# mx-strk/InformationBottleneckDecodingLDPC

Measured on AMD Instinct MI355X. Metric: decoded codewords/sec + achieved HBM GB/s, DVB-S2 N=64800 i_max=50, higher is better.
Workload: dtype u4

## Files before the change

### include/ibldpc.h

```cpp
#ifndef IBLDPC_H
#define IBLDPC_H

#include <stdint.h>

#ifdef __cplusplus
extern "C" {
#endif

#define IBL_VERSION 3

enum { IBL_OK = 0, IBL_EINVAL = -1, IBL_EHIP = -2, IBL_ENOMEM = -3, IBL_EUNSUPPORTED = -4 };
enum { IBL_U8 = 1, IBL_I32 = 2, IBL_F32 = 3, IBL_F64 = 4, IBL_I8 = 5 };
enum { IBL_MINSUM = 0, IBL_BP = 1 };
enum { IBL_PATH_AUTO = 0, IBL_PATH_PASSES = 1, IBL_PATH_FUSED = 2 };
enum { IBL_FLAG_FORCE_GENERIC = 1 };

typedef struct ibl_graph ibl_graph;
typedef struct ibl_ib ibl_ib;
typedef struct ibl_float ibl_float;

int ibl_version(void);
const char* ibl_last_error(void);
int ibl_device_count(int32_t* n);

// ... 6 lines not shown
int ibl_graph_info(const ibl_graph* g, int32_t* n_v, int32_t* n_c, int64_t* n_e, int32_t* d_c_max,
                   int32_t* d_v_max);
void ibl_graph_destroy(ibl_graph* g);

int ibl_ib_create(const ibl_graph* g, int32_t T_ch, int32_t T_dec, int32_t imax,
                  const int32_t* cn_lut, int64_t cn_len, const int32_t* vn_lut, int64_t vn_len,
                  const int32_t* match_cn, int64_t mc_len, const int32_t* match_vn, int64_t mv_len,
                  int32_t match, int32_t max_batch, int32_t flags, ibl_ib** out);
int ibl_ib_path(const ibl_ib* h);
int ibl_ib_set_path(ibl_ib* h, int32_t path);
int ibl_ib_path_in_use(const ibl_ib* h, int32_t* fused);
int ibl_ib_set_small_batch(ibl_ib* h, int32_t max_b);
int ibl_ib_small_batch(const ibl_ib* h, int32_t* max_b);
int ibl_ib_folded(const ibl_ib* h, int32_t* n_folded);
int ibl_ib_set_fold(ibl_ib* h, int32_t on);
int ibl_ib_fused_ncw(const ibl_ib* h, int32_t B, int32_t* ncw);
int ibl_ib_decode(ibl_ib* h, const void* d_ch, int32_t ch_dtype, int32_t B, void* d_out, int32_t out_dtype,
                  int32_t early_stop, int32_t* d_iters, void* stream);
void ibl_ib_destroy(ibl_ib* h);
int ibl_ib_timing(ibl_ib* h, int32_t enable);
int ibl_ib_timing_read(ibl_ib* h, double* cn_ms, int32_t* cn_launches, double* vn_ms, int32_t* vn_launches);

int ibl_float_create(const ibl_graph* g, int32_t kind, int32_t imax, double llr_max, int32_t precision,
                     int32_t max_batch, ibl_float** out);
int ibl_float_decode(ibl_float* h, const void* d_llr, int32_t llr_dtype, int32_t B, void* d_out,
                     int32_t out_dtype, int32_t early_stop, int32_t* d_iters, void* stream);
void ibl_float_destroy(ibl_float* h);
int ibl_float_set_path(ibl_float* h, int32_t path);
int ibl_float_path_in_use(const ibl_float* h, int32_t* fused);
int ibl_float_fused_geometry(const ibl_float* h, int32_t B, int32_t* ngroups, int32_t* grid);
// ... 66 lines not shown
```

### informationbottleneckdecodingldpc_amd/_lib.py

```python
from __future__ import annotations

import ctypes
import os

import numpy as np

_HERE = os.path.dirname(os.path.abspath(__file__))
LIB_PATH = os.environ.get("IBLDPC_LIB") or os.path.join(_HERE, "libibldpc.so")

IBL_OK, IBL_EINVAL, IBL_EHIP, IBL_ENOMEM, IBL_EUNSUPPORTED = 0, -1, -2, -3, -4
IBL_U8, IBL_I32, IBL_F32, IBL_F64, IBL_I8 = 1, 2, 3, 4, 5
IBL_MINSUM, IBL_BP = 0, 1
IBL_FLAG_FORCE_GENERIC = 1
IBL_PATH_AUTO, IBL_PATH_PASSES, IBL_PATH_FUSED = 0, 1, 2

EXPORTS = [
    "ibl_version", "ibl_last_error", "ibl_device_count", "ibl_map_node_connections",
    "ibl_graph_create", "ibl_graph_info", "ibl_graph_destroy",
    "ibl_ib_create", "ibl_ib_path", "ibl_ib_set_path", "ibl_ib_path_in_use", "ibl_ib_fused_ncw", "ibl_ib_decode",
    "ibl_ib_set_small_batch", "ibl_ib_small_batch", "ibl_ib_folded", "ibl_ib_set_fold",
    "ibl_ib_destroy",
    "ibl_float_create", "ibl_float_decode", "ibl_float_destroy", "ibl_count_below",
    "ibl_float_set_path", "ibl_float_path_in_use", "ibl_float_fused_geometry", "ibl_float_folded",
    "ibl_float_input_check",
    "ibl_float_set_small_batch", "ibl_float_small_batch",
    "ibl_float_create_corrected", "ibl_float_correction",
    "ibl_ib_timing", "ibl_ib_timing_read", "ibl_float_timing", "ibl_float_timing_read",
    "ibl_channel_sample",
    "ibl_encoder_create",
    "ibl_encoder_algorithm",
    "ibl_encode",
    "ibl_encoder_destroy",
    "ibl_random_bits",
    "ibl_count_errors",
    "ibl_shard_range", "ibl_comm_unique_id", "ibl_comm_create", "ibl_comm_broadcast", "ibl_comm_allreduce_sum_i64",
# ... 30 lines not shown
    L.ibl_graph_create.argtypes = [_i32, _i32, _i32p, _i32p, _i32, ctypes.POINTER(_vp)]
    L.ibl_graph_info.argtypes = [_vp, ctypes.POINTER(_i32), ctypes.POINTER(_i32), ctypes.POINTER(_i64),
                                 ctypes.POINTER(_i32), ctypes.POINTER(_i32)]
    L.ibl_graph_destroy.argtypes = [_vp]
    L.ibl_graph_destroy.restype = None
    L.ibl_ib_create.argtypes = [_vp, _i32, _i32, _i32, _i32p, _i64, _i32p, _i64, _i32p, _i64, _i32p, _i64,
                                _i32, _i32, _i32, ctypes.POINTER(_vp)]
    L.ibl_ib_path.argtypes = [_vp]
    L.ibl_ib_set_path.argtypes = [_vp, _i32]
    L.ibl_ib_path_in_use.argtypes = [_vp, ctypes.POINTER(_i32)]
    L.ibl_ib_fused_ncw.argtypes = [_vp, _i32, ctypes.POINTER(_i32)]
    L.ibl_ib_set_small_batch.argtypes = [_vp, _i32]
    L.ibl_ib_small_batch.argtypes = [_vp, ctypes.POINTER(_i32)]
    L.ibl_ib_folded.argtypes = [_vp, ctypes.POINTER(_i32)]
    L.ibl_ib_set_fold.argtypes = [_vp, _i32]
    L.ibl_ib_decode.argtypes = [_vp, _vp, _i32, _i32, _vp, _i32, _i32, _vp, _vp]
    L.ibl_ib_destroy.argtypes = [_vp]
    L.ibl_ib_destroy.restype = None
    L.ibl_float_create.argtypes = [_vp, _i32, _i32, ctypes.c_double, _i32, _i32, ctypes.POINTER(_vp)]
    L.ibl_float_decode.argtypes = [_vp, _vp, _i32, _i32, _vp, _i32, _i32, _vp, _vp]
    L.ibl_float_destroy.argtypes = [_vp]
    L.ibl_float_destroy.restype = None
    L.ibl_float_set_path.argtypes = [_vp, _i32]
    L.ibl_float_path_in_use.argtypes = [_vp, ctypes.POINTER(_i32)]
    L.ibl_float_fused_geometry.argtypes = [_vp, _i32, ctypes.POINTER(_i32), ctypes.POINTER(_i32)]
    L.ibl_float_folded.argtypes = [_vp, ctypes.POINTER(_i32)]
    L.ibl_float_set_small_batch.argtypes = [_vp, _i32]
    L.ibl_float_small_batch.argtypes = [_vp, ctypes.POINTER(_i32)]
    L.ibl_float_input_check.argtypes = [_vp, ctypes.POINTER(_i32), _vp]
    L.ibl_float_create_corrected.argtypes = [_vp, ctypes.c_double, ctypes.c_double, _i32, ctypes.c_double, _i32, _i32,
# ... 96 lines not shown
```

### informationbottleneckdecodingldpc_amd/csrc/capi_ib.hip

```cpp
#include <cstring>
#include <functional>

#include "host.h"

using namespace ibl;

struct ibl_ib {
  const ibl_graph* g = nullptr;
  int32_t Tc = 0, T = 0, imax = 0, CM = 0, VM = 0, match = 0, max_batch = 0, ldb = 0;
  bool fast = false;
  DevBuf<uint8_t> cin, vin, ch8;
  DevBuf<int32_t> flags, dL;
  DevBuf<uint32_t> cn_img, vn_img, dec_img;
  int cn_nt = 0, vn_nt = 0, dec_nt = 0;
  int32_t cn_fslot[kMaxD + 1] = {0}, vn_fslot[kMaxD + 1] = {0};
  KCfg kcn, kvn, kdec;
  KTimer timer;
  int32_t n_folded = 0, fold_slot = -1, n_rest = 0, rest_heavy = 0;
  bool fold_on = true;
  std::vector<int32_t> fold_rec, fold_cn_info, fold_vn_info;
  DevBuf<uint8_t> cin2;
  DevBuf<int32_t> fold, cn_info_f, vn_info_r;
  int32_t path = IBL_PATH_AUTO;
  bool fused_ok = false, f_half_ok = false;
  int32_t f_ncw_forced = 0;
  int32_t small_b = 0;
  bool s_ok = false;
  size_t s_lds_cn = 0, s_lds_vn = 0, s_lds_dec = 0;
  ChainGraphs s_graphs;
  FusedTaskBufs ft;
  int32_t f_nreg = 0, f_dbuf = 0, f_cn_uni = 0, f_vn_uni = 0;
  size_t f_lds = 0;
  int f_grid = 0, f_block = 0;
  DevBuf<int32_t> cn_lut, vn_lut, mc, mv;
  int64_t cn_len = 0, vn_len = 0, mc_len = 0, mv_len = 0;
};

// ... 226 lines not shown
  }
  if (const char* ne = getenv("IBL_FUSED_NCW")) h->f_ncw_forced = atoi(ne);
  h->f_nreg = nreg;
  h->f_dbuf = dbuf ? 1 : 0;
  h->f_lds = lds;
  h->f_block = block;
  h->f_grid = bpc * g->num_cus;
  h->fused_ok = true;
  return IBL_OK;
}

int ib_configure_fast(ibl_ib* h, const IbImages& im) {
  const ibl_graph* g = h->g;
  const int CM = h->CM, VM = h->VM;
  int rc;
  if ((rc = h->cn_img.upload(im.cn_img)) || (rc = h->vn_img.upload(im.vn_img)) || (rc = h->dec_img.upload(im.dec_img)))
    return rc;
  if ((rc = pick_cfg(0, CM, 4 * h->cn_nt, g->num_cus, &h->kcn)) ||
      (rc = pick_cfg(1, VM, 4 * h->vn_nt, g->num_cus, &h->kvn)) ||
      (rc = pick_cfg(2, VM, 4 * h->dec_nt, g->num_cus, &h->kdec)))
    return rc;
  size_t priv = 0;
  const char* kname = "";
  HIPCHK(ib_fast_private_bytes(CM, VM, &priv, &kname));
#if IBL_DIAG
  const bool allow_scratch = getenv("IBL_ALLOW_SCRATCH") != nullptr;
#else
  const bool allow_scratch = false;
#endif
  if (!allow_scratch && (rc = refuse_private(priv, std::string("fast-path kernel ") + kname + " has a ",
                                             "-byte private segment (register spill / scratch item): rebuild required")))
    return rc;
// ... 152 lines not shown
  dc.aligned = out_aligned(B, d_out, 4, out_dtype == kU8 ? 1 : 4);
  HIPCHK(launch_ib_dec_small(dc, grid_of(g->n_vn_task, h->s_lds_dec), h->s_lds_dec, s));
  return IBL_OK;
}

int ib_decode_fast(ibl_ib* h, const void* d_ch, int32_t ch_dtype, int32_t B, void* d_out, int32_t out_dtype,
                   bool early, int32_t* d_iters, hipStream_t s) {
  const ibl_graph* g = h->g;
  const int I = h->imax;
  const int ccn = ib_fast_chunk(h->CM), cvn = ib_fast_chunk(h->VM);
  const int ldbb = h->ldb / 2;
  HIPCHK(launch_ib_stage4(d_ch, ch_dtype, g->n_v, B, h->ch8, ldbb, s));
  IbFastArgs cn{}, vn{};
  ib_pass_args(h, B, ldbb, &cn, &vn);
  cn.n_heavy = g->cn_heavy; vn.n_heavy = g->vn_heavy;
  const bool fold = h->fold_on && h->n_folded > 0 && I > 1;
  int rc;
  if (fold) {
    if ((rc = ib_fold_alloc(h))) return rc;
    vn.info = h->vn_info_r; vn.n_nodes = h->n_rest; vn.n_heavy = h->rest_heavy;
    cn.fold = h->fold; cn.fold_slot = h->fold_slot;
  }
  uint8_t* cb[2] = {h->cin, fold ? h->cin2 : h->cin};
  auto cn_fold = [&](int j) {
    const bool f = fold && j < I - 1;
    cn.info = f ? h->cn_info_f.get() : g->cn_info.get();
    cn.fold_mode = f ? ((early && j >= 1) ? 2 : 1) : 0;
    cn.fout = f ? cb[(j + 1) & 1] : nullptr;
  };
#if IBL_DIAG
// ... 20 lines not shown
  const char* trace_path = getenv("IBL_TRACE_WAVES");
  TraceBuf tr;
  nwv = (size_t)h->kvn.grid * (h->kvn.block / 64);
  const size_t nwc = (size_t)h->kcn.grid * (h->kcn.block / 64);
  if (trace_path && I > 1) {
    if ((rc = tr.open(3 * (nwv + nwc), s))) return rc;
    trace = tr.d;
  }
#endif
  for (int j = 1; j < I; ++j) {
    const int32_t* gate = flag_row(h->flags, early && j >= 2, j - 1);
    vn.img = h->vn_img + (size_t)(j - 1) * h->vn_nt * 256;
    vn.gate = gate;
    vn.trace = (trace && j == I / 2) ? trace : nullptr;
    vn.out = cb[j & 1];
    HIPCHK(h->timer.timed(1, s, [&] { return launch_ib_vn_fast(vn, h->VM, h->kvn.grid, h->kvn.block, h->kvn.lds, s); }));
    cn.img = h->cn_img + (size_t)j * h->cn_nt * 256;
    cn.gate = gate;
    cn.unsat = flag_row(h->flags, early, j);
    cn.trace = (trace && j == I / 2) ? trace + 3 * nwv : nullptr;
    cn.in = cb[j & 1];
    cn_fold(j);
    HIPCHK(h->timer.timed(0, s, launch_cn));
  }
#if IBL_DIAG
  if (trace && ((rc = tr.save(s, std::string(trace_path) + "_vn.bin", 0, 3 * nwv)) ||
                (rc = tr.save(s, std::string(trace_path) + "_cn.bin", 3 * nwv, 3 * nwc))))
    return rc;
#endif
  HIPCHK(launch_finalize(h->flags, I, early ? 1 : 0, h->dL, d_iters, s));
  IbDecArgs dc{};
// ... 113 lines not shown
  return IBL_OK;
}

int ibl_ib_folded(const ibl_ib* h, int32_t* n_folded) {
  if (!h || !n_folded) return fail(IBL_EINVAL, "NULL argument");
  *n_folded = h->n_folded;
  return IBL_OK;
}

int ibl_ib_set_fold(ibl_ib* h, int32_t on) {
  if (!h) return fail(IBL_EINVAL, "decoder is NULL");
  h->fold_on = on != 0;
  return IBL_OK;
}

int ibl_ib_timing(ibl_ib* h, int32_t enable) { return timing_enable(h, enable); }
int ibl_ib_timing_read(ibl_ib* h, double* cn_ms, int32_t* cn_n, double* vn_ms, int32_t* vn_n) {
  return timing_read(h, cn_ms, cn_n, vn_ms, vn_n);
}

void ibl_ib_destroy(ibl_ib* h) {
  if (h) (void)hipSetDevice(h->g->device);
  delete h;
}

int ibl_ib_decode(ibl_ib* h, const void* d_ch, int32_t ch_dtype, int32_t B, void* d_out, int32_t out_dtype,
                  int32_t early_stop, int32_t* d_iters, void* stream) {
  if (!h) return fail(IBL_EINVAL, "decoder is NULL");
  if (B < 1 || B > h->max_batch) return fail(IBL_EINVAL, "B must lie in [1, max_batch]");
  if (ch_dtype != kU8 && ch_dtype != kI32) return fail(IBL_EINVAL, "channel dtype must be IBL_U8 or IBL_I32");
// ... 14 lines not shown
```

### informationbottleneckdecodingldpc_amd/csrc/common.h

```cpp
#pragma once
#include <hip/hip_runtime.h>
#pragma clang diagnostic ignored "-Wunused-result"
#include <stddef.h>
#include <stdint.h>

#include "plan.h"

namespace ibl {

constexpr int kWave = 64;
constexpr int kChunk = 256;
#ifndef IBL_W
#define IBL_W 2
#endif
constexpr int kW = IBL_W;
constexpr int kChunkIB = 512 * kW;
#ifndef IBL_LIGHT_W
#define IBL_LIGHT_W 4
#endif
constexpr int kRowPad = 512 * (IBL_LIGHT_W > IBL_W ? IBL_LIGHT_W : IBL_W);
constexpr int kChunkDec = 512;
constexpr int kTbl = 8192;
constexpr int kSuper = 65536;
constexpr int kRowSh = 12, kColSh = 8;
// ... 5 lines not shown
constexpr int kShards = 64;
constexpr int kLdsBytes = 160 * 1024;

enum Dtype : int32_t { kU8 = 1, kI32 = 2, kF32 = 3, kF64 = 4, kI8 = 5 };

int set_error(int code, const char* msg);

typedef __attribute__((address_space(4))) const int32_t cint32;
__device__ __forceinline__ int32_t sload(const int32_t* p, int i) { return ((cint32*)p)[i]; }

__device__ __forceinline__ int take_ticket(int* ctr, int lane) {
  int t = 0;
  if (lane == 0) t = __hip_atomic_fetch_add(ctr, 1, __ATOMIC_RELAXED, __HIP_MEMORY_SCOPE_WORKGROUP);
  return __builtin_amdgcn_readfirstlane(t);
}

struct IbFastArgs {
  const uint8_t* in;
  uint8_t* out;
  const uint8_t* ch8;
  const int32_t* info;
  const int32_t* tgt;
  const int32_t* gather;
  const uint32_t* img;
  const int32_t* gate;
  int32_t* unsat;
  int32_t fslot[kMaxD + 1];
  int32_t nt;
  int32_t n_nodes, nchunks, ldb, B, half, match;
  int32_t n_heavy;
  uint64_t* trace;
  const int32_t* task;
  int32_t n_tasks, nwords;
  const int32_t* fold;
  uint8_t* fout;
  int32_t fold_mode, fold_slot;
};

struct IbDecArgs {
  const uint8_t* vin;
  const uint8_t* ch8;
  const int32_t* start;
  const int32_t* deg;
  const uint32_t* img;
  const int32_t* iters;
  void* out;
  int32_t out_dtype, nt, n_nodes, nchunks, ldb, B, aligned;
  const int32_t* info;
  const int32_t* task;
  int32_t n_tasks, nwords;
};

// ... 95 lines not shown
  const void* vin1;
  const void* ch;
  const int32_t* start;
  const int32_t* deg;
  const int32_t* iters;
  void* out;
  int32_t out_dtype, n_nodes, nchunks, ldb, B, aligned;
  const int32_t* info;
  const int32_t* task;
  int32_t n_tasks, nwords;
};

hipError_t launch_ib_stage(const void* ch, int dtype, int n, int B, uint8_t* ch8, int ldb, hipStream_t s);
hipError_t launch_ib_stage4(const void* ch, int dtype, int n, int B, uint8_t* ch4, int ldb_bytes, hipStream_t s);
hipError_t launch_ib_cn_fast(const IbFastArgs& a, int maxd, int grid, int block, size_t lds, hipStream_t s);
hipError_t launch_ib_vn_fast(const IbFastArgs& a, int maxd, int grid, int block, size_t lds, hipStream_t s);
int ib_fast_chunk(int maxd);
hipError_t launch_ib_dec_fast(const IbDecArgs& a, int grid, int block, size_t lds, hipStream_t s);
constexpr int kSmallBlock = 1024;
__host__ __device__ constexpr int small_block(int nwords) { return nwords <= 1 ? 256 : (nwords <= 8 ? 512 : 1024); }
constexpr int kFlSmallBlock = 256;
constexpr int kSmallBatchDefault = 224;
constexpr int kFlSmallBatchDefault = 64;
hipError_t launch_ib_cn_small(const IbFastArgs& a, int maxd, int grid, size_t lds, hipStream_t s);
hipError_t launch_ib_vn_small(const IbFastArgs& a, int maxd, int grid, size_t lds, hipStream_t s);
hipError_t launch_ib_dec_small(const IbDecArgs& a, int grid, size_t lds, hipStream_t s);
hipError_t ib_small_private_bytes(int cn_maxd, int vn_maxd, size_t* bytes, const char** name);
hipError_t ib_fast_occupancy(int which, int maxd, int block, size_t lds, int* blocks_per_cu);
hipError_t ib_fast_private_bytes(int cn_maxd, int vn_maxd, size_t* bytes, const char** name);
hipError_t launch_ib_stage_t(const void* ch, int dtype, int n, int B, const int32_t* perm, uint32_t* chT,
                             hipStream_t s);
// ... 127 lines not shown
```

### informationbottleneckdecodingldpc_amd/csrc/ib_kernels.hip

```cpp
#include <algorithm>

#include "common.h"

namespace ibl {


typedef __attribute__((address_space(3))) const uint8_t lds8_t;
__device__ __forceinline__ uint32_t lu(uint32_t x, uint32_t c) {
  asm("" : "+v"(x));
  return *(lds8_t*)(size_t)(x + c);
}
__device__ __forceinline__ uint32_t luc(uint32_t t, uint32_t q, uint32_t c) {
  uint32_t x;
  static_assert(kRowSh == 12, "luc's shift is the row shift of the table layout");
  asm("v_lshl_or_b32 %0, %1, 12, %2" : "=v"(x) : "v"(t), "v"(q));
  return *(lds8_t*)(size_t)(x + c);
}
__device__ __forceinline__ uint32_t lds_base(const uint8_t* p) { return (uint32_t)(size_t)(lds8_t*)p; }
__device__ __forceinline__ void lds_at_zero(const uint8_t* lds) {
  if (lds_base(lds) != 0u) __builtin_trap();
}

__device__ __forceinline__ uint32_t qidx(uint32_t m, uint32_t lane4) { return (m << kColSh) | lane4; }

// ... 490 lines not shown
#pragma unroll
    for (int s = 0; s < 4; ++s) {
      const int k = 4 * g + s;
      uint32_t Q = lu((nib(cw, k) << kRowSh) + qidx(nib(inw[0], k), lane4), 0);
#pragma unroll
      for (int l = 1; l < D; ++l) Q = luc(Q, qidx(nib(inw[l], k), lane4), slot_off(l));
      packed |= Q << (8 * s);
    }
    store4(a.out, a.out_dtype, (size_t)node * a.B, cwb + 4 * g, a.B, a.aligned != 0, packed);
  }
}

#define IBL_DEG_CASES(X) X(2) X(3) X(4) X(5) X(6) X(7) X(8) X(9) X(10) X(11) X(12) X(13) X(14) X(15) X(16)
#define IBL_DEG_CASES8(X) X(2) X(3) X(4) X(5) X(6) X(7) X(8)

__device__ __forceinline__ int* lds_counters(const uint8_t* lds, const IbFastArgs& a) {
  return reinterpret_cast<int*>(const_cast<uint8_t*>(lds) + lds_of_quads(a.nt));
}
__device__ __forceinline__ void stage_pass(uint8_t* lds, const IbFastArgs& a) {
  if (threadIdx.x < 2) lds_counters(lds, a)[threadIdx.x] = 0;
  stage_tables(lds, a.img, a.nt);
}

#ifndef IBL_LIGHT_DEPTH
#define IBL_LIGHT_DEPTH 2
#endif
template <class Buf, bool VN, bool GATHER, int DLO, int DEPTH = 2, int FOLD = 0>
__device__ __forceinline__ void ib_phase(const IbFastArgs& a, uint32_t lane4, int lane, int first,
                                         int end, int nw, int wpb, int* ctr, bool do_par, bool& unsat,
                                         uint64_t* trace_items, const PhaseItems pi) {
  auto compute = [&](const Buf& cur) __attribute__((always_inline)) {
    settle<VN>(cur);
    if constexpr (VN) {
      switch (cur.d) {
        case 1: if constexpr (DLO < 1) vn_compute<1>(a, lane4, cur, 0); break;
#define X(D) case D: if constexpr (D > DLO && D <= Buf::kMax) vn_compute<D>(a, lane4, cur, a.fslot[D]); break;
        IBL_DEG_CASES(X)
#undef X
        default: break;
      }
    } else {
      switch (cur.d) {
#define X(D) case D: if constexpr (D > DLO && D <= Buf::kMax) { \
          if constexpr (FOLD != 0) cn_compute_fold<D, GATHER, FOLD == 2>(a, lane4, cur, a.fslot[D], do_par, unsat); \
          else cn_compute<D, GATHER>(a, lane4, cur, a.fslot[D], do_par, unsat); } break;
        IBL_DEG_CASES(X)
#undef X
        default: break;
      }
    }
  };
  const int base = first + (int)blockIdx.x * wpb;
  auto item_of = [&](int k) { return base + (k % wpb) + nw * (k / wpb); };
  int done = 0;
  if constexpr (DEPTH == 3) {
    Buf A, Bb, Cc;
    int ia = item_of(take_ticket(ctr, lane));
    if (ia >= end) return;
    fetch_item<Buf, VN, GATHER, FOLD>(a, ia, lane, A, pi);
    int ib = item_of(take_ticket(ctr, lane));
    fetch_item<Buf, VN, GATHER, FOLD>(a, min(ib, end - 1), lane, Bb, pi);
    int kn = take_ticket(ctr, lane);
    for (;;) {
      int ic = item_of(kn);
      fetch_item<Buf, VN, GATHER, FOLD>(a, min(ic, end - 1), lane, Cc, pi);
      kn = take_ticket(ctr, lane);
      compute(A);
      ++done;
      if (ib >= end) break;
      ia = item_of(kn);
      fetch_item<Buf, VN, GATHER, FOLD>(a, min(ia, end - 1), lane, A, pi);
      kn = take_ticket(ctr, lane);
      compute(Bb);
      ++done;
      if (ic >= end) break;
      ib = item_of(kn);
      fetch_item<Buf, VN, GATHER, FOLD>(a, min(ib, end - 1), lane, Bb, pi);
      kn = take_ticket(ctr, lane);
      compute(Cc);
      ++done;
      if (ia >= end) break;
    }
  } else {
    Buf A, Bb;
    int item = item_of(take_ticket(ctr, lane));
    if (item >= end) return;
    fetch_item<Buf, VN, GATHER, FOLD>(a, item, lane, A, pi);
    int kn = take_ticket(ctr, lane);
    for (;;) {
      int next = item_of(kn);
      fetch_item<Buf, VN, GATHER, FOLD>(a, min(next, end - 1), lane, Bb, pi);
      kn = take_ticket(ctr, lane);
      compute(A);
      ++done;
      if (next >= end) break;
      item = next;
      next = item_of(kn);
      fetch_item<Buf, VN, GATHER, FOLD>(a, min(next, end - 1), lane, A, pi);
      kn = take_ticket(ctr, lane);
      compute(Bb);
      ++done;
      if (next >= end) break;
      item = next;
    }
  }
  if (trace_items && lane == 0) *trace_items += (uint64_t)done;
}

template <int MAXD, bool VN, bool GATHER, int FOLD = 0>
__device__ __forceinline__ void ib_pass(const IbFastArgs& a, const uint8_t* lds) {
  const int lane = threadIdx.x & 63;
  const uint32_t lane4 = (uint32_t)(lane & 31) << 2;
  const int wpb = blockDim.x >> 6;
  const int gw = __builtin_amdgcn_readfirstlane(blockIdx.x * wpb + (threadIdx.x >> 6)), nw = gridDim.x * wpb;
  constexpr int W = rowW<MAXD>();
  constexpr int LW = (VN && MAXD <= 8) ? IBL_LIGHT_W : W;
  const int nch_l = LW == W ? a.nchunks : (a.B + 512 * LW - 1) / (512 * LW);
  const int heavy_end = a.n_heavy * a.nchunks, nitems = heavy_end + (a.n_nodes - a.n_heavy) * nch_l;
  const bool do_par = !VN && !GATHER && a.unsat != nullptr;
  bool unsat = false;
  uint64_t* trace_items = a.trace ? a.trace + 3 * gw + 2 : nullptr;
  if (a.trace && lane == 0) {
    a.trace[3 * gw] = __builtin_readcyclecounter();
    *trace_items = (uint64_t)__smid() << 32;
  }
  int* ctr = lds_counters(lds, a);
#ifndef IBL_MIX16
#define IBL_MIX16 6
#endif
  const bool light_first = VN && (int)(threadIdx.x >> 6) * 16 < wpb * IBL_MIX16;
#pragma unroll 1
  for (int r = 0; r < 2; ++r) {
    if ((r == 0) != light_first)
      ib_phase<ItemBuf<MAXD, W>, VN, GATHER, kLightD, 2, FOLD>(a, lane4, lane, 0, heavy_end, nw, wpb, ctr, do_par, unsat,
                                                      trace_items, PhaseItems{0, 0, a.nchunks});
    else
      ib_phase<ItemBuf<kLightD, LW>, VN, GATHER, 0, (VN ? IBL_LIGHT_DEPTH : 2), FOLD>(a, lane4, lane, heavy_end, nitems, nw, wpb, ctr + 1, do_par,
                                                   unsat, trace_items, PhaseItems{heavy_end, a.n_heavy, nch_l});
  }
  if (a.trace && lane == 0) {
    a.trace[3 * gw + 1] = __builtin_readcyclecounter();
  }
  if (do_par && unsat && lane == 0) atomicOr(&a.unsat[gw & (kShards - 1)], 1);
}

#ifndef IBL_LB8
#define IBL_LB8 1024
#endif
#ifndef IBL_LB16
#define IBL_LB16 512
#endif
#ifndef IBL_WPE8
#define IBL_WPE8 1
#endif
#ifndef IBL_LB8C
#define IBL_LB8C IBL_LB8
#endif
#ifndef IBL_WPE8C
#define IBL_WPE8C IBL_WPE8
#endif
template <int MAXD, bool GATHER, int FOLD = 0>
__global__ __launch_bounds__(MAXD <= 8 ? IBL_LB8C : IBL_LB16, MAXD <= 8 ? IBL_WPE8C : 1) void ib_cn_fast(IbFastArgs a) {
  static_assert(FOLD == 0 || MAXD <= 8, "the max-degree-16 bodies do not fold");
  extern __shared__ __attribute__((aligned(16))) uint8_t lds[];
  if (!gate_open(a.gate, threadIdx.x & 63)) return;
  lds_at_zero(lds);
  stage_pass(lds, a);
  __syncthreads();
  ib_pass<MAXD, false, GATHER, FOLD>(a, lds);
}

template <int MAXD>
__global__ __launch_bounds__(MAXD <= 8 ? IBL_LB8 : IBL_LB16, MAXD <= 8 ? IBL_WPE8 : 1) void ib_vn_fast(IbFastArgs a) {
  extern __shared__ __attribute__((aligned(16))) uint8_t lds[];
  if (!gate_open(a.gate, threadIdx.x & 63)) return;
  lds_at_zero(lds);
  stage_pass(lds, a);
  __syncthreads();
  ib_pass<MAXD, true, false>(a, lds);
}

__global__ __launch_bounds__(1024) void ib_dec_fast(IbDecArgs a) {
  extern __shared__ __attribute__((aligned(16))) uint8_t lds[];
  const int lane = threadIdx.x & 63;
  const int L = __builtin_amdgcn_readfirstlane(*a.iters);
  lds_at_zero(lds);
  stage_tables(lds, a.img + (size_t)L * a.nt * 256, a.nt);
  __syncthreads();
  const uint32_t lane4 = (uint32_t)(lane & 31) << 2;
  const int wpb = blockDim.x >> 6;
  const int gw = blockIdx.x * wpb + (threadIdx.x >> 6), nw = gridDim.x * wpb;
  const int nitems = a.n_nodes * a.nchunks;
  for (int item = gw; item < nitems; item += nw) {
    const int node = __builtin_amdgcn_readfirstlane(item / a.nchunks);
// ... 840 lines not shown
    if (!ib_fold_args_ok(a, maxd)) return hipErrorInvalidValue;
    if (a.gather) hipLaunchKernelGGL((ib_cn_fast<8, true, 1>), dim3(grid), dim3(block), lds, s, a);
    else if (a.fold_mode == 2) hipLaunchKernelGGL((ib_cn_fast<8, false, 2>), dim3(grid), dim3(block), lds, s, a);
    else hipLaunchKernelGGL((ib_cn_fast<8, false, 1>), dim3(grid), dim3(block), lds, s, a);
    return hipGetLastError();
  }
  if (a.gather) {
    if (maxd <= 8) hipLaunchKernelGGL((ib_cn_fast<8, true>), dim3(grid), dim3(block), lds, s, a);
    else hipLaunchKernelGGL((ib_cn_fast<16, true>), dim3(grid), dim3(block), lds, s, a);
  } else {
    if (maxd <= 8) hipLaunchKernelGGL((ib_cn_fast<8, false>), dim3(grid), dim3(block), lds, s, a);
    else hipLaunchKernelGGL((ib_cn_fast<16, false>), dim3(grid), dim3(block), lds, s, a);
  }
  return hipGetLastError();
}
hipError_t launch_ib_vn_fast(const IbFastArgs& a, int maxd, int grid, int block, size_t lds, hipStream_t s) {
  if (maxd <= 8) hipLaunchKernelGGL(ib_vn_fast<8>, dim3(grid), dim3(block), lds, s, a);
  else hipLaunchKernelGGL(ib_vn_fast<16>, dim3(grid), dim3(block), lds, s, a);
  return hipGetLastError();
}
int ib_fast_chunk(int maxd) { return maxd <= 8 ? chunkOf<8>() : chunkOf<16>(); }
static bool ib_small_args_ok(const IbFastArgs& a, bool vn) {
  return a.task && a.info && a.tgt && a.out && a.img && a.ch8 && (a.in || (!vn && a.gather)) && a.n_tasks >= 0 &&
         a.nwords >= 1 && 4 * a.nwords <= a.ldb;
}
hipError_t launch_ib_cn_small(const IbFastArgs& a, int maxd, int grid, size_t lds, hipStream_t s) {
  if (!ib_small_args_ok(a, false)) return hipErrorInvalidValue;
  if (a.gather) {
    if (maxd <= 8) hipLaunchKernelGGL((ib_cn_small<8, true>), dim3(grid), dim3(small_block(a.nwords)), lds, s, a);
    else hipLaunchKernelGGL((ib_cn_small<16, true>), dim3(grid), dim3(small_block(a.nwords)), lds, s, a);
  } else {
    if (maxd <= 8) hipLaunchKernelGGL((ib_cn_small<8, false>), dim3(grid), dim3(small_block(a.nwords)), lds, s, a);
    else hipLaunchKernelGGL((ib_cn_small<16, false>), dim3(grid), dim3(small_block(a.nwords)), lds, s, a);
// ... 140 lines not shown
```

### informationbottleneckdecodingldpc_amd/csrc/plan.h

```cpp
#pragma once
#include <stddef.h>
#include <stdint.h>

#include <algorithm>
#include <string>
#include <vector>

namespace ibl {

constexpr int kMaxD = 16;
constexpr int kLightD = 4;
constexpr int kFoldRec = 8;

struct HostGraph {
  int32_t n_v = 0, n_c = 0;
  int64_t n_e = 0;
  std::vector<int32_t> h_cn_deg, h_vn_deg;
  std::vector<int32_t> h_cn_start, h_cols, h_vn_start, h_tgt_vn;
};

inline bool map_node_connections(int32_t n_v, int32_t n_c, const int32_t* indptr, const int32_t* cols,
                                 int32_t* cn_start, int32_t* cn_deg, int32_t* tgt_cn, int32_t* vn_start,
                                 int32_t* vn_deg, int32_t* tgt_vn, std::string* err) {
  if (n_v <= 0 || n_c <= 0 || !indptr || !cols) return *err = "empty graph", false;
// ... 360 lines not shown
      pl->dir = -1;
      pl->order = piv;
    }
  }
  bool chain = true;
  for (int i = 0; i < M && chain; ++i) {
    const int n = pl->P.ip[i + 1] - pl->P.ip[i];
    const int want = pl->dir > 0 ? i - 1 : i + 1;
    if (want < 0 || want >= M) chain = n == 0;
    else chain = n == 1 && pl->P.ix[pl->P.ip[i]] == want;
  }
  pl->chain = chain ? 1 : 0;
  return 0;
}

}
```

### informationbottleneckdecodingldpc_amd/engine.py

```python
from __future__ import annotations

import ctypes
from typing import Optional

import numpy as np
import torch

from . import _lib
from .graph import EdgeGraph, build_graph
from .tables import IBTables

_DT_IB = {torch.uint8: _lib.IBL_U8, torch.int32: _lib.IBL_I32}
_DT_FL = {torch.float32: _lib.IBL_F32, torch.float64: _lib.IBL_F64}
_DT_ANY = {torch.uint8: _lib.IBL_U8, torch.int32: _lib.IBL_I32, torch.float32: _lib.IBL_F32,
           torch.float64: _lib.IBL_F64}


def _require_gpu(device) -> torch.device:
    if not torch.cuda.is_available():
        raise RuntimeError("no HIP device visible: the LDPC decoders run only on the GPU (no CPU fallback)")
    dev = torch.device("cuda", torch.cuda.current_device()) if device is None else torch.device(device)
    if dev.type != "cuda":
        raise ValueError(f"decoder device must be a HIP (cuda) device, got {dev}")
    if dev.index is None:
# ... 32 lines not shown
    def __del__(self):
        h = getattr(self, "_h", None)
        if h is not None and h.value:
            try:
                _lib.load().ibl_graph_destroy(h)
            except Exception:
                pass
            self._h = None


class IBDecoder:

    _PATHS = {"auto": _lib.IBL_PATH_AUTO, "passes": _lib.IBL_PATH_PASSES, "fused": _lib.IBL_PATH_FUSED}

    def __init__(self, graph: Graph, tables: IBTables, match: bool, max_batch: int, force_generic: bool = False,
                 path: str = "auto", fold: bool = True):
        self.graph = graph
        self.tables = tables
        self.match = bool(match)
        self.max_batch = int(max_batch)
        self.device = graph.device
        tb = tables
        cn = np.ascontiguousarray(tb.cn, np.int32)
        vn = np.ascontiguousarray(tb.vn, np.int32)
        mc = np.ascontiguousarray(tb.match_cn if tb.match_cn is not None else np.zeros(1), np.int32)
        mv = np.ascontiguousarray(tb.match_vn if tb.match_vn is not None else np.zeros(1), np.int32)
        h = ctypes.c_void_p()
        L = _lib.load()
        _lib.check(L.ibl_ib_create(graph.handle, tb.Tc, tb.T, tb.imax, cn, cn.size, vn, vn.size, mc, mc.size,
                                   mv, mv.size, int(self.match), self.max_batch,
                                   _lib.IBL_FLAG_FORCE_GENERIC if force_generic else 0, ctypes.byref(h)),
                   "ibl_ib_create")
        self._h = h
        self.fast_path = bool(L.ibl_ib_path(h))
        if path not in self._PATHS:
            raise ValueError(f"path must be one of {sorted(self._PATHS)}")
        _lib.check(L.ibl_ib_set_path(h, self._PATHS[path]), "ibl_ib_set_path")
        if not fold:
            self.fold = False

    @property
    def fused(self) -> bool:
        f = ctypes.c_int32()
        _lib.check(_lib.load().ibl_ib_path_in_use(self._h, ctypes.byref(f)), "ibl_ib_path_in_use")
        return bool(f.value)

    @property
    def small_batch(self) -> int:
        n = ctypes.c_int32()
        _lib.check(_lib.load().ibl_ib_small_batch(self._h, ctypes.byref(n)), "ibl_ib_small_batch")
        return int(n.value)

    @small_batch.setter
    def small_batch(self, max_b: int) -> None:
# ... 1 lines not shown

    @property
    def folded(self) -> int:
        f = ctypes.c_int32()
        _lib.check(_lib.load().ibl_ib_folded(self._h, ctypes.byref(f)), "ibl_ib_folded")
        return int(f.value)

    @property
    def fold(self) -> bool:
        return getattr(self, "_fold", True)

    @fold.setter
    def fold(self, on: bool) -> None:
        _lib.check(_lib.load().ibl_ib_set_fold(self._h, int(bool(on))), "ibl_ib_set_fold")
        self._fold = bool(on)

    def fused_ncw(self, B: int) -> int:
        n = ctypes.c_int32()
        _lib.check(_lib.load().ibl_ib_fused_ncw(self._h, int(B), ctypes.byref(n)), "ibl_ib_fused_ncw")
        return int(n.value)

    def decode(self, ch: torch.Tensor, out: Optional[torch.Tensor] = None, out_dtype=torch.int32,
               early_stop: bool = True, iters: Optional[torch.Tensor] = None) -> torch.Tensor:
        n = self.graph.edges.n_v
        _check_tensor(ch, self.device, n, "channel values")
        if ch.dtype not in _DT_IB:
            raise ValueError("channel values must be uint8 or int32")
        B = ch.shape[1]
        if out is None:
            out = torch.empty((n, B), dtype=out_dtype, device=self.device)
# ... 402 lines not shown
```

Before: 203,300.

## Add cross-block work stealing for the tail of the VN pass

Splits each VN phase into a static per-block round-robin portion and a tail (default 2/16 of rounds) that blocks claim dynamically through a global atomic counter, so blocks that finish early take the leftover items. The goal is to cut load imbalance at the end of each VN launch. It adds a per-iteration memset, global atomics and spin-wait logic in LDS counters. It also raises launch-bounds waves per EU for the degree-16 VN kernel from 1 to 4, which may change register allocation.

```diff
diff --git a/include/ibldpc.h b/include/ibldpc.h
--- a/include/ibldpc.h
+++ b/include/ibldpc.h
@@ -44,6 +44,8 @@
 int ibl_ib_small_batch(const ibl_ib* h, int32_t* max_b);
 int ibl_ib_folded(const ibl_ib* h, int32_t* n_folded);
 int ibl_ib_set_fold(ibl_ib* h, int32_t on);
+int ibl_ib_set_steal(ibl_ib* h, int32_t sixteenths);
+int ibl_ib_steal(const ibl_ib* h, int32_t* sixteenths);
 int ibl_ib_fused_ncw(const ibl_ib* h, int32_t B, int32_t* ncw);
 int ibl_ib_decode(ibl_ib* h, const void* d_ch, int32_t ch_dtype, int32_t B, void* d_out, int32_t out_dtype,
                   int32_t early_stop, int32_t* d_iters, void* stream);
diff --git a/informationbottleneckdecodingldpc_amd/_lib.py b/informationbottleneckdecodingldpc_amd/_lib.py
--- a/informationbottleneckdecodingldpc_amd/_lib.py
+++ b/informationbottleneckdecodingldpc_amd/_lib.py
@@ -19,6 +19,7 @@
     "ibl_graph_create", "ibl_graph_info", "ibl_graph_destroy",
     "ibl_ib_create", "ibl_ib_path", "ibl_ib_set_path", "ibl_ib_path_in_use", "ibl_ib_fused_ncw", "ibl_ib_decode",
     "ibl_ib_set_small_batch", "ibl_ib_small_batch", "ibl_ib_folded", "ibl_ib_set_fold",
+    "ibl_ib_set_steal", "ibl_ib_steal",
     "ibl_ib_destroy",
     "ibl_float_create", "ibl_float_decode", "ibl_float_destroy", "ibl_count_below",
     "ibl_float_set_path", "ibl_float_path_in_use", "ibl_float_fused_geometry", "ibl_float_folded",
@@ -79,6 +80,8 @@
     L.ibl_ib_small_batch.argtypes = [_vp, ctypes.POINTER(_i32)]
     L.ibl_ib_folded.argtypes = [_vp, ctypes.POINTER(_i32)]
     L.ibl_ib_set_fold.argtypes = [_vp, _i32]
+    L.ibl_ib_set_steal.argtypes = [_vp, _i32]
+    L.ibl_ib_steal.argtypes = [_vp, ctypes.POINTER(_i32)]
     L.ibl_ib_decode.argtypes = [_vp, _vp, _i32, _i32, _vp, _i32, _i32, _vp, _vp]
     L.ibl_ib_destroy.argtypes = [_vp]
     L.ibl_ib_destroy.restype = None
diff --git a/informationbottleneckdecodingldpc_amd/csrc/capi_ib.hip b/informationbottleneckdecodingldpc_amd/csrc/capi_ib.hip
--- a/informationbottleneckdecodingldpc_amd/csrc/capi_ib.hip
+++ b/informationbottleneckdecodingldpc_amd/csrc/capi_ib.hip
@@ -4,6 +4,8 @@
 #include "host.h"
 
 using namespace ibl;
+
+constexpr int32_t kStealDefault = 2;
 
 struct ibl_ib {
   const ibl_graph* g = nullptr;
@@ -21,6 +23,8 @@
   std::vector<int32_t> fold_rec, fold_cn_info, fold_vn_info;
   DevBuf<uint8_t> cin2;
   DevBuf<int32_t> fold, cn_info_f, vn_info_r;
+  int32_t steal16 = kStealDefault;
+  DevBuf<int32_t> steal;
   int32_t path = IBL_PATH_AUTO;
   bool fused_ok = false, f_half_ok = false;
   int32_t f_ncw_forced = 0;
@@ -277,8 +281,11 @@
   const ibl_graph* g = h->g;
   const int CM = h->CM, VM = h->VM;
   int rc;
-  if ((rc = h->cn_img.upload(im.cn_img)) || (rc = h->vn_img.upload(im.vn_img)) || (rc = h->dec_img.upload(im.dec_img)))
+  if ((rc = h->cn_img.upload(im.cn_img)) || (rc = h->vn_img.upload(im.vn_img)) || (rc = h->dec_img.upload(im.dec_img)) ||
+      (rc = h->steal.alloc_zero((size_t)2 * h->imax)))
     return rc;
+  if (const char* st = getenv("IBL_STEAL"))
+    h->steal16 = std::min(16, std::max(0, atoi(st)));
   if ((rc = pick_cfg(0, CM, 4 * h->cn_nt, g->num_cus, &h->kcn)) ||
       (rc = pick_cfg(1, VM, 4 * h->vn_nt, g->num_cus, &h->kvn)) ||
       (rc = pick_cfg(2, VM, 4 * h->dec_nt, g->num_cus, &h->kdec)))
@@ -461,6 +468,7 @@
   IbFastArgs cn{}, vn{};
   ib_pass_args(h, B, ldbb, &cn, &vn);
   cn.n_heavy = g->cn_heavy; vn.n_heavy = g->vn_heavy;
+  if (h->steal16 > 0) HIPCHK(hipMemsetAsync(h->steal, 0, sizeof(int32_t) * 2 * (size_t)I, s));
   const bool fold = h->fold_on && h->n_folded > 0 && I > 1;
   int rc;
   if (fold) {
@@ -511,7 +519,7 @@
     vn.gate = gate;
     vn.trace = (trace && j == I / 2) ? trace : nullptr;
     vn.out = cb[j & 1];
-    HIPCHK(h->timer.timed(1, s, [&] { return launch_ib_vn_fast(vn, h->VM, h->kvn.grid, h->kvn.block, h->kvn.lds, s); }));
+    HIPCHK(h->timer.timed(1, s, [&] { return launch_ib_vn_fast(vn, h->steal16, h->steal + 2 * (size_t)j, h->VM, h->kvn.grid, h->kvn.block, h->kvn.lds, s); }));
     cn.img = h->cn_img + (size_t)j * h->cn_nt * 256;
     cn.gate = gate;
     cn.unsat = flag_row(h->flags, early, j);
@@ -655,6 +663,19 @@
   return IBL_OK;
 }
 
+int ibl_ib_set_steal(ibl_ib* h, int32_t sixteenths) {
+  if (sixteenths < 0 || sixteenths > 16) return fail(IBL_EINVAL, "tail sixteenths must lie in [0, 16]");
+  if (!h) return fail(IBL_EINVAL, "decoder is NULL");
+  h->steal16 = sixteenths;
+  return IBL_OK;
+}
+
+int ibl_ib_steal(const ibl_ib* h, int32_t* sixteenths) {
+  if (!h || !sixteenths) return fail(IBL_EINVAL, "NULL argument");
+  *sixteenths = h->steal16;
+  return IBL_OK;
+}
+
 int ibl_ib_timing(ibl_ib* h, int32_t enable) { return timing_enable(h, enable); }
 int ibl_ib_timing_read(ibl_ib* h, double* cn_ms, int32_t* cn_n, double* vn_ms, int32_t* vn_n) {
   return timing_read(h, cn_ms, cn_n, vn_ms, vn_n);
diff --git a/informationbottleneckdecodingldpc_amd/csrc/common.h b/informationbottleneckdecodingldpc_amd/csrc/common.h
--- a/informationbottleneckdecodingldpc_amd/csrc/common.h
+++ b/informationbottleneckdecodingldpc_amd/csrc/common.h
@@ -43,6 +43,11 @@
   if (lane == 0) t = __hip_atomic_fetch_add(ctr, 1, __ATOMIC_RELAXED, __HIP_MEMORY_SCOPE_WORKGROUP);
   return __builtin_amdgcn_readfirstlane(t);
 }
+__device__ __forceinline__ int take_global_ticket(int32_t* ctr, int lane) {
+  int t = 0;
+  if (lane == 0) t = __hip_atomic_fetch_add(ctr, 1, __ATOMIC_RELAXED, __HIP_MEMORY_SCOPE_AGENT);
+  return __builtin_amdgcn_readfirstlane(t);
+}
 
 struct IbFastArgs {
   const uint8_t* in;
@@ -65,6 +70,10 @@
   uint8_t* fout;
   int32_t fold_mode, fold_slot;
 };
+struct IbStealArgs {
+  int32_t* ctr;
+  int32_t srounds[2], tfirst[2], trounds[2];
+};
 
 struct IbDecArgs {
   const uint8_t* vin;
@@ -190,7 +199,8 @@
 hipError_t launch_ib_stage(const void* ch, int dtype, int n, int B, uint8_t* ch8, int ldb, hipStream_t s);
 hipError_t launch_ib_stage4(const void* ch, int dtype, int n, int B, uint8_t* ch4, int ldb_bytes, hipStream_t s);
 hipError_t launch_ib_cn_fast(const IbFastArgs& a, int maxd, int grid, int block, size_t lds, hipStream_t s);
-hipError_t launch_ib_vn_fast(const IbFastArgs& a, int maxd, int grid, int block, size_t lds, hipStream_t s);
+hipError_t launch_ib_vn_fast(const IbFastArgs& a, int steal16, int32_t* ctr, int maxd, int grid, int block, size_t lds,
+                             hipStream_t s);
 int ib_fast_chunk(int maxd);
 hipError_t launch_ib_dec_fast(const IbDecArgs& a, int grid, int block, size_t lds, hipStream_t s);
 constexpr int kSmallBlock = 1024;
diff --git a/informationbottleneckdecodingldpc_amd/csrc/ib_kernels.hip b/informationbottleneckdecodingldpc_amd/csrc/ib_kernels.hip
--- a/informationbottleneckdecodingldpc_amd/csrc/ib_kernels.hip
+++ b/informationbottleneckdecodingldpc_amd/csrc/ib_kernels.hip
@@ -528,6 +528,9 @@
 #define IBL_DEG_CASES(X) X(2) X(3) X(4) X(5) X(6) X(7) X(8) X(9) X(10) X(11) X(12) X(13) X(14) X(15) X(16)
 #define IBL_DEG_CASES8(X) X(2) X(3) X(4) X(5) X(6) X(7) X(8)
 
+constexpr int kNxFirst = -2;
+constexpr int kNxPending = -1;
+constexpr int kCtrTw = 2, kCtrNx = 6, kCtrTail = 8;
 __device__ __forceinline__ int* lds_counters(const uint8_t* lds, const IbFastArgs& a) {
   return reinterpret_cast<int*>(const_cast<uint8_t*>(lds) + lds_of_quads(a.nt));
 }
@@ -535,13 +538,33 @@
   if (threadIdx.x < 2) lds_counters(lds, a)[threadIdx.x] = 0;
   stage_tables(lds, a.img, a.nt);
 }
+__device__ __forceinline__ void stage_pass(uint8_t* lds, const IbFastArgs& a, const IbStealArgs& st) {
+  if (threadIdx.x < 16) {
+    const int t = threadIdx.x;
+    const uint64_t g0 = (uint64_t)(uintptr_t)st.ctr, g1 = (uint64_t)(uintptr_t)(st.ctr + 1);
+    int v = 0;
+    if (t == 2 || t == 4) v = blockDim.x >> 6;
+    if (t == 6) v = st.srounds[0] > 0 ? kNxPending : kNxFirst;
+    if (t == 7) v = st.srounds[1] > 0 ? kNxPending : kNxFirst;
+    if (t == 8) v = (int)(uint32_t)g0;
+    if (t == 9) v = (int)(uint32_t)(g0 >> 32);
+    if (t == 10) v = st.tfirst[0];
+    if (t == 11) v = st.trounds[0];
+    if (t == 12) v = (int)(uint32_t)g1;
+    if (t == 13) v = (int)(uint32_t)(g1 >> 32);
+    if (t == 14) v = st.tfirst[1];
+    if (t == 15) v = st.trounds[1];
+    lds_counters(lds, a)[t] = v;
+  }
+  stage_tables(lds, a.img, a.nt);
+}
 
 #ifndef IBL_LIGHT_DEPTH
 #define IBL_LIGHT_DEPTH 2
 #endif
-template <class Buf, bool VN, bool GATHER, int DLO, int DEPTH = 2, int FOLD = 0>
+template <class Buf, bool VN, bool GATHER, int DLO, int DEPTH = 2, int FOLD = 0, int P = 0>
 __device__ __forceinline__ void ib_phase(const IbFastArgs& a, uint32_t lane4, int lane, int first,
-                                         int end, int nw, int wpb, int* ctr, bool do_par, bool& unsat,
+                                         int end, int nw, int wpb, int* c, int srounds, bool do_par, bool& unsat,
                                          uint64_t* trace_items, const PhaseItems pi) {
   auto compute = [&](const Buf& cur) __attribute__((always_inline)) {
     settle<VN>(cur);
@@ -564,54 +587,107 @@
       }
     }
   };
-  const int base = first + (int)blockIdx.x * wpb;
-  auto item_of = [&](int k) { return base + (k % wpb) + nw * (k / wpb); };
+  constexpr int kLeft = INT32_MIN;
+  int sp = (srounds - 1) * wpb;
+  auto ctr_load = [&](int i) __attribute__((always_inline)) -> int {
+    return __builtin_amdgcn_readfirstlane(__hip_atomic_load(c + i, __ATOMIC_RELAXED, __HIP_MEMORY_SCOPE_WORKGROUP));
+  };
+  auto ctr_store = [&](int i, int v) __attribute__((always_inline)) {
+    if (lane == 0) __hip_atomic_store(c + i, v, __ATOMIC_RELAXED, __HIP_MEMORY_SCOPE_WORKGROUP);
+  };
+  auto global_take = [&]() __attribute__((always_inline)) -> int {
+    const uint64_t g = (uint64_t)(uint32_t)ctr_load(kCtrTail + 4 * P) | (uint64_t)(uint32_t)ctr_load(kCtrTail + 4 * P + 1) << 32;
+    return take_global_ticket(reinterpret_cast<int32_t*>((uintptr_t)g), lane);
+  };
+  auto tail_take = [&]() __attribute__((always_inline)) -> int {
+    unsigned long long* tw = reinterpret_cast<unsigned long long*>(c + kCtrTw + 2 * P);
+    for (;;) {
+      unsigned long long o = 0;
+      if (lane == 0) o = __hip_atomic_fetch_add(tw, 1ull, __ATOMIC_RELAXED, __HIP_MEMORY_SCOPE_WORKGROUP);
+      const int w = __builtin_amdgcn_readfirstlane((int)(uint32_t)o);
+      const int it = __builtin_amdgcn_readfirstlane((int)(uint32_t)(o >> 32));
+      if (w < wpb) return it + w;
+      if (w == wpb) {
+        int v;
+        for (;;) {
+          v = ctr_load(kCtrNx + P);
+          if (v != kNxPending) break;
+          __builtin_amdgcn_s_sleep(1);
+        }
+        const int tn = v == kNxFirst ? global_take() : v;
+        const bool more = tn < ctr_load(kCtrTail + 4 * P + 3);
+        const int it0 = more ? ctr_load(kCtrTail + 4 * P + 2) + tn * wpb : end;
+        ctr_store(kCtrNx + P, more ? kNxPending : tn);
+        if (lane == 0)
+          __hip_atomic_store(tw, ((unsigned long long)(uint32_t)it0 << 32) | 1ull, __ATOMIC_RELEASE,
+                             __HIP_MEMORY_SCOPE_WORKGROUP);
+        if (more) ctr_store(kCtrNx + P, global_take());
+        return it0;
+      }
+      __builtin_amdgcn_s_sleep(1);
+    }
+  };
+  auto take = [&]() __attribute__((always_inline)) -> int {
+    if constexpr (!VN) return take_ticket(c + P, lane);
+    if (sp != kLeft) {
+      const int k = take_ticket(c + P, lane);
+      if (k < sp) return k;
+      if (k == sp) ctr_store(kCtrNx + P, global_take());
+      if (k < sp + wpb) return k;
+      sp = kLeft;
+    }
+    return ~tail_take();
+  };
+  auto item_of = [&](int k) __attribute__((always_inline)) -> int {
+    if constexpr (!VN) return ib_static_item(first, (int)blockIdx.x, wpb, nw, k);
+    return k >= 0 ? ib_static_item(first, (int)blockIdx.x, wpb, nw, k) : ~k;
+  };
   int done = 0;
   if constexpr (DEPTH == 3) {
     Buf A, Bb, Cc;
-    int ia = item_of(take_ticket(ctr, lane));
+    int ia = item_of(take());
     if (ia >= end) return;
     fetch_item<Buf, VN, GATHER, FOLD>(a, ia, lane, A, pi);
-    int ib = item_of(take_ticket(ctr, lane));
+    int ib = item_of(take());
     fetch_item<Buf, VN, GATHER, FOLD>(a, min(ib, end - 1), lane, Bb, pi);
-    int kn = take_ticket(ctr, lane);
+    int kn = take();
     for (;;) {
       int ic = item_of(kn);
       fetch_item<Buf, VN, GATHER, FOLD>(a, min(ic, end - 1), lane, Cc, pi);
-      kn = take_ticket(ctr, lane);
+      kn = take();
       compute(A);
       ++done;
       if (ib >= end) break;
       ia = item_of(kn);
       fetch_item<Buf, VN, GATHER, FOLD>(a, min(ia, end - 1), lane, A, pi);
-      kn = take_ticket(ctr, lane);
+      kn = take();
       compute(Bb);
       ++done;
       if (ic >= end) break;
       ib = item_of(kn);
       fetch_item<Buf, VN, GATHER, FOLD>(a, min(ib, end - 1), lane, Bb, pi);
-      kn = take_ticket(ctr, lane);
+      kn = take();
       compute(Cc);
       ++done;
       if (ia >= end) break;
     }
   } else {
     Buf A, Bb;
-    int item = item_of(take_ticket(ctr, lane));
+    int item = item_of(take());
     if (item >= end) return;
     fetch_item<Buf, VN, GATHER, FOLD>(a, item, lane, A, pi);
-    int kn = take_ticket(ctr, lane);
+    int kn = take();
     for (;;) {
       int next = item_of(kn);
       fetch_item<Buf, VN, GATHER, FOLD>(a, min(next, end - 1), lane, Bb, pi);
-      kn = take_ticket(ctr, lane);
+      kn = take();
       compute(A);
       ++done;
       if (next >= end) break;
       item = next;
       next = item_of(kn);
       fetch_item<Buf, VN, GATHER, FOLD>(a, min(next, end - 1), lane, A, pi);
-      kn = take_ticket(ctr, lane);
+      kn = take();
       compute(Bb);
       ++done;
       if (next >= end) break;
@@ -622,7 +698,7 @@
 }
 
 template <int MAXD, bool VN, bool GATHER, int FOLD = 0>
-__device__ __forceinline__ void ib_pass(const IbFastArgs& a, const uint8_t* lds) {
+__device__ __forceinline__ void ib_pass(const IbFastArgs& a, const uint8_t* lds, const int (&srounds)[2]) {
   const int lane = threadIdx.x & 63;
   const uint32_t lane4 = (uint32_t)(lane & 31) << 2;
   const int wpb = blockDim.x >> 6;
@@ -646,10 +722,10 @@
 #pragma unroll 1
   for (int r = 0; r < 2; ++r) {
     if ((r == 0) != light_first)
-      ib_phase<ItemBuf<MAXD, W>, VN, GATHER, kLightD, 2, FOLD>(a, lane4, lane, 0, heavy_end, nw, wpb, ctr, do_par, unsat,
+      ib_phase<ItemBuf<MAXD, W>, VN, GATHER, kLightD, 2, FOLD, 0>(a, lane4, lane, 0, heavy_end, nw, wpb, ctr, srounds[0], do_par, unsat,
                                                       trace_items, PhaseItems{0, 0, a.nchunks});
     else
-      ib_phase<ItemBuf<kLightD, LW>, VN, GATHER, 0, (VN ? IBL_LIGHT_DEPTH : 2), FOLD>(a, lane4, lane, heavy_end, nitems, nw, wpb, ctr + 1, do_par,
+      ib_phase<ItemBuf<kLightD, LW>, VN, GATHER, 0, (VN ? IBL_LIGHT_DEPTH : 2), FOLD, 1>(a, lane4, lane, heavy_end, nitems, nw, wpb, ctr, srounds[1], do_par,
                                                    unsat, trace_items, PhaseItems{heavy_end, a.n_heavy, nch_l});
   }
   if (a.trace && lane == 0) {
@@ -666,6 +742,9 @@
 #endif
 #ifndef IBL_WPE8
 #define IBL_WPE8 1
+#endif
+#ifndef IBL_WPE16
+#define IBL_WPE16 4
 #endif
 #ifndef IBL_LB8C
 #define IBL_LB8C IBL_LB8
@@ -681,17 +760,17 @@
   lds_at_zero(lds);
   stage_pass(lds, a);
   __syncthreads();
-  ib_pass<MAXD, false, GATHER, FOLD>(a, lds);
+  ib_pass<MAXD, false, GATHER, FOLD>(a, lds, {kIbAllStatic, kIbAllStatic});
 }
 
 template <int MAXD>
-__global__ __launch_bounds__(MAXD <= 8 ? IBL_LB8 : IBL_LB16, MAXD <= 8 ? IBL_WPE8 : 1) void ib_vn_fast(IbFastArgs a) {
+__global__ __launch_bounds__(MAXD <= 8 ? IBL_LB8 : IBL_LB16, MAXD <= 8 ? IBL_WPE8 : IBL_WPE16) void ib_vn_fast(IbFastArgs a, IbStealArgs st) {
   extern __shared__ __attribute__((aligned(16))) uint8_t lds[];
   if (!gate_open(a.gate, threadIdx.x & 63)) return;
   lds_at_zero(lds);
-  stage_pass(lds, a);
+  stage_pass(lds, a, st);
   __syncthreads();
-  ib_pass<MAXD, true, false>(a, lds);
+  ib_pass<MAXD, true, false>(a, lds, st.srounds);
 }
 
 __global__ __launch_bounds__(1024) void ib_dec_fast(IbDecArgs a) {
@@ -1562,9 +1641,23 @@
   }
   return hipGetLastError();
 }
-hipError_t launch_ib_vn_fast(const IbFastArgs& a, int maxd, int grid, int block, size_t lds, hipStream_t s) {
-  if (maxd <= 8) hipLaunchKernelGGL(ib_vn_fast<8>, dim3(grid), dim3(block), lds, s, a);
-  else hipLaunchKernelGGL(ib_vn_fast<16>, dim3(grid), dim3(block), lds, s, a);
+hipError_t launch_ib_vn_fast(const IbFastArgs& a, int steal16, int32_t* ctr, int maxd, int grid, int block, size_t lds,
+                             hipStream_t s) {
+  if (steal16 < 0 || steal16 > 16 || (steal16 > 0 && !ctr)) return hipErrorInvalidValue;
+  const int w = maxd <= 8 ? rowW<8>() : rowW<16>(), lw = maxd <= 8 ? IBL_LIGHT_W : w;
+  const int nch_l = lw == w ? a.nchunks : (a.B + 512 * lw - 1) / (512 * lw);
+  const int nw = grid * (block / 64);
+  const int bound[3] = {0, a.n_heavy * a.nchunks, a.n_heavy * a.nchunks + (a.n_nodes - a.n_heavy) * nch_l};
+  IbStealArgs st{};
+  st.ctr = ctr;
+  for (int p = 0; p < 2; ++p) {
+    st.srounds[p] = ib_static_rounds(bound[p + 1] - bound[p], nw, steal16);
+    const IbTail t = ib_tail_of(bound[p], bound[p + 1], nw, block / 64, st.srounds[p]);
+    st.tfirst[p] = t.first;
+    st.trounds[p] = t.rounds;
+  }
+  if (maxd <= 8) hipLaunchKernelGGL(ib_vn_fast<8>, dim3(grid), dim3(block), lds, s, a, st);
+  else hipLaunchKernelGGL(ib_vn_fast<16>, dim3(grid), dim3(block), lds, s, a, st);
   return hipGetLastError();
 }
 int ib_fast_chunk(int maxd) { return maxd <= 8 ? chunkOf<8>() : chunkOf<16>(); }
diff --git a/informationbottleneckdecodingldpc_amd/csrc/plan.h b/informationbottleneckdecodingldpc_amd/csrc/plan.h
--- a/informationbottleneckdecodingldpc_amd/csrc/plan.h
+++ b/informationbottleneckdecodingldpc_amd/csrc/plan.h
@@ -398,4 +398,19 @@
   return 0;
 }
 
-}
+constexpr int32_t kIbAllStatic = INT32_MAX / 64;
+constexpr int32_t ib_static_rounds(int32_t n_items, int32_t nw, int32_t sixteenths) {
+  return sixteenths <= 0 || nw <= 0 ? kIbAllStatic : (int32_t)((int64_t)(n_items / nw) * (16 - sixteenths) / 16);
+}
+constexpr int32_t ib_static_item(int32_t first, int32_t block, int32_t wpb, int32_t nw, int32_t k) {
+  return first + block * wpb + k % wpb + nw * (k / wpb);
+}
+struct IbTail {
+  int32_t first, rounds;
+};
+constexpr IbTail ib_tail_of(int32_t first, int32_t end, int32_t nw, int32_t wpb, int32_t srounds) {
+  const int64_t tf = (int64_t)first + (int64_t)srounds * nw;
+  return tf >= end ? IbTail{end, 0} : IbTail{(int32_t)tf, (int32_t)((end - tf + wpb - 1) / wpb)};
+}
+
+}
diff --git a/informationbottleneckdecodingldpc_amd/engine.py b/informationbottleneckdecodingldpc_amd/engine.py
--- a/informationbottleneckdecodingldpc_amd/engine.py
+++ b/informationbottleneckdecodingldpc_amd/engine.py
@@ -70,7 +70,7 @@
     _PATHS = {"auto": _lib.IBL_PATH_AUTO, "passes": _lib.IBL_PATH_PASSES, "fused": _lib.IBL_PATH_FUSED}
 
     def __init__(self, graph: Graph, tables: IBTables, match: bool, max_batch: int, force_generic: bool = False,
-                 path: str = "auto", fold: bool = True):
+                 path: str = "auto", fold: bool = True, steal: Optional[int] = None):
         self.graph = graph
         self.tables = tables
         self.match = bool(match)
@@ -94,6 +94,8 @@
         _lib.check(L.ibl_ib_set_path(h, self._PATHS[path]), "ibl_ib_set_path")
         if not fold:
             self.fold = False
+        if steal is not None:
+            self.steal = steal
 
     @property
     def fused(self) -> bool:
@@ -125,6 +127,16 @@
     def fold(self, on: bool) -> None:
         _lib.check(_lib.load().ibl_ib_set_fold(self._h, int(bool(on))), "ibl_ib_set_fold")
         self._fold = bool(on)
+
+    @property
+    def steal(self) -> int:
+        n = ctypes.c_int32()
+        _lib.check(_lib.load().ibl_ib_steal(self._h, ctypes.byref(n)), "ibl_ib_steal")
+        return int(n.value)
+
+    @steal.setter
+    def steal(self, sixteenths: int) -> None:
+        _lib.check(_lib.load().ibl_ib_set_steal(self._h, int(sixteenths)), "ibl_ib_set_steal")
 
     def fused_ncw(self, B: int) -> int:
         n = ctypes.c_int32()
```

Result: no change. 204,300 (median of 6 runs) (+0.5%).
